# AlgoLab/rs-vgaligner

Measured on AMD Instinct MI355X. Metric: aligned reads/sec (10 kbp ONT vs HLA graph), higher is better.
Workload: dtype int32+f64

## Files before the change

rs-vgaligner_amd/csrc/vga_poa_t5.hpp:

```cpp
#pragma once

template <int B>
__device__ __forceinline__ void t5_min_byte(int &dst, int t, int c)
{
    if constexpr (B == 0) asm("v_min_u32_sdwa %0, %1, %2 dst_sel:BYTE_0 dst_unused:UNUSED_PRESERVE src0_sel:DWORD src1_sel:DWORD" : "+v"(dst) : "v"(t), "s"(c));
    if constexpr (B == 1) asm("v_min_u32_sdwa %0, %1, %2 dst_sel:BYTE_1 dst_unused:UNUSED_PRESERVE src0_sel:DWORD src1_sel:DWORD" : "+v"(dst) : "v"(t), "s"(c));
    if constexpr (B == 2) asm("v_min_u32_sdwa %0, %1, %2 dst_sel:BYTE_2 dst_unused:UNUSED_PRESERVE src0_sel:DWORD src1_sel:DWORD" : "+v"(dst) : "v"(t), "s"(c));
    if constexpr (B == 3) asm("v_min_u32_sdwa %0, %1, %2 dst_sel:BYTE_3 dst_unused:UNUSED_PRESERVE src0_sel:DWORD src1_sel:DWORD" : "+v"(dst) : "v"(t), "s"(c));
}
__device__ __forceinline__ uint64_t t5_uniform64(uint64_t v)
{
    return ((uint64_t)(uint32_t)__builtin_amdgcn_readfirstlane((int)(v >> 32)) << 32) | (uint32_t)__builtin_amdgcn_readfirstlane((int)(uint32_t)v);
}

__device__ __forceinline__ int t5_own(int v)
{
    asm volatile("" : "+v"(v));
    return __builtin_amdgcn_readfirstlane(v);
}
__device__ __forceinline__ uint32_t t5_own(uint32_t v) { return (uint32_t)t5_own((int)v); }
__device__ __forceinline__ uint64_t t5_own(uint64_t v) { return ((uint64_t)t5_own((uint32_t)(v >> 32)) << 32) | t5_own((uint32_t)v); }
template <typename T>
__device__ __forceinline__ T *t5_own(T *p) { return (T *)t5_own((uint64_t)p); }

#define POA_T5_ARGS_OFFSET 40
__device__ __forceinline__ const poa_t5_args *t5_kargs()
{
    uint32_t off = POA_T5_ARGS_OFFSET;
    asm volatile("" : "+s"(off));
    return (const poa_t5_args *)((const char *)__builtin_amdgcn_kernarg_segment_ptr() + off);
}
template <int NT, bool DEF>
__global__ __launch_bounds__(NT) __attribute__((amdgpu_waves_per_eu(5)))
void k_poa_dp_t5(const poa_prob *__restrict__ probs, const char *__restrict__ queries,
                                                       const uint4 *__restrict__ node_tab, const uint32_t *__restrict__ seq32,
                                                       const uint32_t *__restrict__ preds, const poa_t5_args A)
{
    poa_row *rows = A.rows;
    uint8_t *pool_arg = A.pool;
    const uint32_t lds_cols = t5_own(A.lds_cols), hg_cols = t5_own(A.hg_cols), win_mask = t5_own(A.win_mask);
    enum : uint32_t { ST_CHUNKED = 1u, ST_QPLAIN = 2u, ST_FAILED = 4u, ST_PREV_LDS = 8u, ST_PREV_FAR_USE = 16u };
    uint32_t st = (A.cp.n_slots != 0 ? ST_CHUNKED : 0u) | ST_PREV_LDS;
#define chunked ((st & ST_CHUNKED) != 0)
#define failed ((st & ST_FAILED) != 0)
#define q_plain ((st & ST_QPLAIN) != 0)
#define prev_lds ((st & ST_PREV_LDS) != 0)
#define prev_far_use ((st & ST_PREV_FAR_USE) != 0)
    struct { int match, mismatch, o1, e1, o2, e2, banded; } P = {t5_own(A.P.match), t5_own(A.P.mismatch), A.P.o1, A.P.e1, A.P.o2, A.P.e2, t5_own(A.P.banded)};
    constexpr int NW = NT / 64;
    constexpr int STEP = NT * 4;
    extern __shared__ __attribute__((aligned(16))) uint8_t smem[];
    int4 *sX = (int4 *)smem;
    int4 *sRed = sX + 2 * NW;
    int32_t *edgeW = (int32_t *)(sRed + NW);
    int32_t *sSink = edgeW + 4;
    uint64_t *sChunk = (uint64_t *)(sSink + 4);
    constexpr int HDR = (3 * NW + 1 + 1 + 2) * 16;
    int32_t *Hs = (int32_t *)(smem + HDR);
    uint16_t *Gs = (uint16_t *)(smem + HDR + 4ull * hg_cols);
    uint16_t *Qn = (uint16_t *)(smem + HDR + 6ull * hg_cols);
    const int edge_idx = (int)(edgeW - Hs);

    if (threadIdx.x == 0) A.outs[blockIdx.x].t_begin = __builtin_amdgcn_s_memrealtime();
    if (A.prio) __builtin_amdgcn_s_setprio(3);
    const poa_prob pb = probs[blockIdx.x];
    const int tid = threadIdx.x, lane = tid & 63, wv = __builtin_amdgcn_readfirstlane(tid >> 6);
    const int qlen = t5_own((int)pb.qlen);
    const char *query = queries + pb.q0;
    const uint4 *ntab = node_tab + t5_own(pb.node0);
    const uint32_t *plist = preds + t5_own(pb.pred0);
    const uint32_t *seqw = seq32 + t5_own(pb.seq0 >> 2);
    poa_row *R = rows + t5_own(pb.row0);
    const uint32_t n_nodes = t5_own(pb.n_nodes), ring_rows = t5_own(pb.ring_rows);

    uint8_t *pool = pool_arg;
    uint64_t state_lo = 0, state_hi = 0;
    if (chunked) {
        int got = -1;
        if (!(pb.flags & 1u)) {
            if (tid == 0) {
                got = poa_slot_acquire(A.cp.slot_flag, A.cp.n_slots, blockIdx.x);
                sSink[1] = got;
            }
            __syncthreads();
            got = __builtin_amdgcn_readfirstlane(sSink[1]);
        }
        if (got < 0) {
            if (tid == 0) {
                poa_out &O = A.outs[blockIdx.x];
                O.t_end = O.t_begin; O.cells = 0; O.vcells = 0; O.maxw = 0; O.nops = 0;
                O.score = POA_NEG; O.row = 0; O.status = POA_ST_POOL;
            }
            return;
        }
        __builtin_amdgcn_fence(__ATOMIC_ACQUIRE, "agent");
        pool = nullptr;
        state_lo = (uint64_t)A.cp.state_base + (uint64_t)(uint32_t)got * A.cp.state_size;
        state_hi = state_lo + A.cp.state_size;
    }

    const int o1 = DEF ? 4 : P.o1, e1 = DEF ? 2 : P.e1, o2 = DEF ? 24 : P.o2, e2 = DEF ? 1 : P.e2;
    const int C1 = 4 * (o1 + e1), C2 = 4 * (o2 + e2) + 1;
    const int D1 = 4 * o1, D2 = 4 * o2 + 1;
    const uint32_t g_bias = (uint32_t)(4 * e1 | (4 * e2) << 8) * 0x00010001u;
    const uint32_t e_probe = (uint32_t)((128 - D1) | (128 - D2) << 8) * 0x00010001u;
    const int bw = t5_own((int)pb.w);

    uint32_t own_head = POA_NIL, own_chunks = 0;
    auto alloc = [&](uint64_t &cur, uint32_t &rem, uint32_t bytes_asked, int slot) -> uint64_t {
        const uint32_t bytes = (bytes_asked + 15u) & ~15u;
        if (__builtin_expect(bytes > rem, 0)) {
            if (chunked) {
                if (slot == 0 && bytes <= POA_CHUNK) {
                    const poa_t5_args *ka = t5_kargs();
                    if (tid == 0) {
                        const uint32_t idx = poa_chunk_pop(ka->cp, blockIdx.x);
                        if (idx != POA_NIL) __hip_atomic_store(ka->cp.next + idx, own_head, __ATOMIC_RELAXED, __HIP_MEMORY_SCOPE_AGENT);
                        if (own_chunks == 0) sChunk[3] = idx;
                        sChunk[0] = idx;
                    }
                    __syncthreads();
                    const uint32_t idx = (uint32_t)__builtin_amdgcn_readfirstlane((int)(uint32_t)sChunk[0]);
                    __syncthreads();
                    if (idx == POA_NIL) st |= ST_FAILED;
// ... 70 lines not shown
        asm volatile("" : "+s"(st));
        POA_MARK("row_topo");
        const uint32_t r = nt.x + tn;
        const bool last = tn + 1 == nlen;
        const bool is_sink = last && (nt.z >> 31) != 0;
        const uint32_t ps = nt.w;
        uint32_t gb = 0;
        if (v > 0) {
            const uint32_t bi = r - 1;
            if ((bi & 3u) == 0 || (bi >> 2) != seq_word_idx) { seq_word_idx = bi >> 2; seq_word = seqw[seq_word_idx]; }
            gb = (seq_word >> (8u * (bi & 3u))) & 0xffu;
        }
        const bool simple = r > 0 && prev_lds && (tn > 0 || ((nt.y >> 24) == 1u && ps == r - 1));
        const bool writer = wv == (int)(r % (uint32_t)NW);
        POA_MARK("row_prevmax");
        int prev_lmax = 0, prev_rmax = 0;
        if (r > 0) {
            int4 rw = make_int4(INT32_MIN, INT32_MAX, INT32_MIN, 0);
            if (lane < NW) rw = sRed[lane];
            int b = rw.x, t;
            t = poa_dpp<0x111, 0xf>(INT32_MIN, b); b = t > b ? t : b;
            if (NW > 2) { t = poa_dpp<0x112, 0xf>(INT32_MIN, b); b = t > b ? t : b; }
            if (NW > 4) { t = poa_dpp<0x114, 0xf>(INT32_MIN, b); b = t > b ? t : b; }
            if (NW > 8) { t = poa_dpp<0x118, 0xf>(INT32_MIN, b); b = t > b ? t : b; }
            const int rbest = __builtin_amdgcn_readlane(b, NW - 1);
            const uint64_t tie = __builtin_amdgcn_ballot_w64(rw.x == rbest);
            if (__builtin_expect(__builtin_popcountll(tie) == 1, 1)) {
                const int w1 = __builtin_ctzll(tie);
                prev_lmax = __builtin_amdgcn_readlane(rw.y, w1);
                prev_rmax = __builtin_amdgcn_readlane(rw.z, w1);
            } else {
                int lm = rw.x == rbest ? rw.y : INT32_MAX, rm = rw.x == rbest ? rw.z : INT32_MIN;
                t = poa_dpp<0x111, 0xf>(INT32_MAX, lm); lm = t < lm ? t : lm;
                t = poa_dpp<0x111, 0xf>(INT32_MIN, rm); rm = t > rm ? t : rm;
                if (NW > 2) {
                    t = poa_dpp<0x112, 0xf>(INT32_MAX, lm); lm = t < lm ? t : lm;
                    t = poa_dpp<0x112, 0xf>(INT32_MIN, rm); rm = t > rm ? t : rm;
                }
                if (NW > 4) {
                    t = poa_dpp<0x114, 0xf>(INT32_MAX, lm); lm = t < lm ? t : lm;
                    t = poa_dpp<0x114, 0xf>(INT32_MIN, rm); rm = t > rm ? t : rm;
                }
                if (NW > 8) {
                    t = poa_dpp<0x118, 0xf>(INT32_MAX, lm); lm = t < lm ? t : lm;
                    t = poa_dpp<0x118, 0xf>(INT32_MIN, rm); rm = t > rm ? t : rm;
                }
                prev_lmax = __builtin_amdgcn_readlane(lm, NW - 1);
                prev_rmax = __builtin_amdgcn_readlane(rm, NW - 1);
            }
            if (prev_far_use && writer && lane == 0) { R[r - 1].lmax = prev_lmax; R[r - 1].rmax = prev_rmax; }
        }
        POA_MARK("row_setup");
        const int remain = (int)(nt.z & 0x3fffffffu) + (int)(nlen - 1 - tn);
        int beg, end, np, pbeg = prev_beg, pend = prev_end;
        bool first, single, sp_near;
        uint32_t sp = r - 1;
        uint64_t vpo = 0;
        if (__builtin_expect(simple, 1)) {
            first = tn == 0;
            np = 1; single = true; sp_near = true;
            const int mpl = prev_lmax + 1, mpr = prev_rmax + 1;
            if (!P.banded) { beg = 0; end = qlen; }
            else {
                const int diag = qlen - remain;
                const int lo = mpl < diag ? mpl : diag;
                const int hi = mpr > diag ? mpr : diag;
                beg = lo - bw; if (beg < 0) beg = 0;
                end = hi + bw; if (end > qlen) end = qlen;
            }
        } else {
            first = tn == 0 && v > 0;
            np = v == 0 ? 0 : (tn == 0 ? (int)(nt.y >> 24) : 1);
            bool far = r > 0 && !prev_lds;
            if (first) {
                if (np == 1) far |= ps != r - 1;
                else
                    for (int t = 0; t < np; t++) far |= plist[ps + t] != r - 1;
            }
            single = r > 0 && np == 1;
            sp = first ? ps : r - 1;
            sp_near = sp == r - 1 && prev_lds;
            if (far) __syncthreads();
            int mpl, mpr;
            if (r == 0) { mpl = 0; mpr = 0; }
            else if (!first) { mpl = prev_lmax + 1; mpr = prev_rmax + 1; }
            else {
                mpl = INT32_MAX; mpr = 0;
                for (int t = 0; t < np; t++) {
                    const uint32_t p = np == 1 ? ps : plist[ps + t];
                    int lm, rm;
                    if (p == r - 1) { lm = prev_lmax + 1; rm = prev_rmax + 1; }
                    else {
                        lm = __builtin_amdgcn_readfirstlane(R[p].lmax) + 1;
                        rm = __builtin_amdgcn_readfirstlane(R[p].rmax) + 1;
                    }
                    mpl = lm < mpl ? lm : mpl;
                    mpr = rm > mpr ? rm : mpr;
                }
            }
            if (!P.banded) { beg = 0; end = qlen; }
            else {
                const int diag = qlen - remain;
                const int lo = mpl < diag ? mpl : diag;
                const int hi = mpr > diag ? mpr : diag;
                beg = lo - bw; if (beg < 0) beg = 0;
                end = hi + bw; if (end > qlen) end = qlen;
            }
            if (single && !sp_near) {
                pbeg = __builtin_amdgcn_readfirstlane(R[sp].beg);
                pend = __builtin_amdgcn_readfirstlane(R[sp].end);
                vpo = t5_uniform64(R[sp].voff);
            }
        }
        const int bal = beg & ~3;
        const int W = (end - bal + 1 + 3) & ~3;
        const bool wide = (uint32_t)W + 8u > hg_cols;
        const bool keep = last || wide;
        const uint64_t doff = alloc(dcur, dend, (uint32_t)W * (np > 1 ? 4u : 1u), 0);
        uint64_t voff = 0;
        if (last && !failed) {
            if (r == 0 || (nt.z & 0x40000000u)) voff = chunked ? alloc(dcur, dend, 6u * (uint32_t)W, 0) : alloc(vcur, vendp, 6u * (uint32_t)W, 1);
            else {
                voff = ring_base + (uint64_t)ring_head * ((6u * (uint32_t)((qlen + 8) & ~3) + 15u) & ~15u);
                ring_head = ring_head + 1 == ring_rows ? 0 : ring_head + 1;
            }
        } else if (wide) voff = wide_scratch + (r & 1u) * 6ull * lds_cols;
        if (__builtin_expect(failed, 0)) break;
        if (writer && lane == 0) {
            uint32_t *rec = (uint32_t *)(R + r);
            *(uint4 *)rec = make_uint4((uint32_t)beg, (uint32_t)end, (uint32_t)doff, (uint32_t)(doff >> 32));
            *(uint2 *)(rec + 4) = make_uint2((uint32_t)voff, (uint32_t)(voff >> 32));
            *(HIP_vector_type<uint32_t, 3> *)(rec + 8) = HIP_vector_type<uint32_t, 3>(ps, first ? (uint32_t)np : 0u, keep ? 1u : 0u);
        }
        uint8_t *Vrow = pool + voff;
        uint8_t *drow = pool + doff;
        const uint32_t gd = gb - (uint32_t)'A';
        const bool acgt = gd < 20u && ((0x80045u >> gd) & 1u);
        const int sc_eq = acgt ? P.match : 0, sc_ne = acgt ? -P.mismatch : 0;
        const int gsh = (int)((gb >> 1) & 3u);
        const int ne4t = 4 * sc_ne + 1, mm4 = 4 * (sc_eq - sc_ne);
        const bool staged = !simple && r > 0 && !wide && q_plain;
        if (staged) {
            POA_MARK("row_stage");
            if (chunked) {
                bool no_row = false;
                for (int t = 0; t < np; t++) no_row |= t5_uniform64(R[np == 1 ? sp : plist[ps + t]].voff) == 0;
                if (__builtin_expect(no_row, 0)) st |= ST_FAILED;
            }
            for (int c0 = 0; c0 < W; c0 += STEP) {
                const int c = c0 + 4 * tid;
                const int j0 = bal + c;
                if (j0 <= end && np == 1) {
                    const int bp = __builtin_amdgcn_readfirstlane(R[sp].beg), ep = __builtin_amdgcn_readfirstlane(R[sp].end);
                    const uint64_t vq_off = t5_uniform64(R[sp].voff);
                    const uint8_t *Vq = pool + vq_off;
                    const bool vq_ok = !chunked || vq_off != 0;
                    const int balq = bp & ~3;
                    const int Wq = (ep - balq + 1 + 3) & ~3;
                    const int idx = j0 - balq;
                    int4 hv = make_int4(T4_NEG, T4_NEG, T4_NEG, T4_NEG);
                    uint2 gg = make_uint2(0u, 0u);
                    if (idx >= 0 && idx < Wq && vq_ok) {
                        hv = *(const int4 *)((const int32_t *)Vq + idx);
                        gg = *(const uint2 *)(Vq + 4ll * Wq + 2ll * idx);
                    }
                    const unsigned pspan = (unsigned)(ep - bp);
                    const bool in0 = (unsigned)(j0 - bp) <= pspan, in1 = (unsigned)(j0 + 1 - bp) <= pspan, in2 = (unsigned)(j0 + 2 - bp) <= pspan,
                               in3 = (unsigned)(j0 + 3 - bp) <= pspan;
                    hv.x = in0 ? hv.x : T4_NEG; hv.y = in1 ? hv.y : T4_NEG; hv.z = in2 ? hv.z : T4_NEG; hv.w = in3 ? hv.w : T4_NEG;
                    gg.x = (in0 ? gg.x & 0xffffu : 0u) | (in1 ? gg.x & 0xffff0000u : 0u);
                    gg.y = (in2 ? gg.y & 0xffffu : 0u) | (in3 ? gg.y & 0xffff0000u : 0u);
                    *(int4 *)(Hs + (j0 & win_mask)) = hv;
                    *(uint2 *)(Gs + (j0 & win_mask)) = gg;
                    if (c == 0 && bal > 0) {
                        const int wl = (idx >= 1 && idx - 1 < Wq && vq_ok) ? ((const int32_t *)Vq)[idx - 1] : 0;
                        Hs[(bal - 1) & win_mask] = (unsigned)(j0 - 1 - bp) <= pspan ? wl : T4_NEG;
                    }
                } else if (j0 <= end) {
                    int hm[4], x1[4], x2[4], ah[4], a1[4], a2[4];
                    int hl = T4_NEG, ahl = 0;
#pragma unroll
                    for (int k = 0; k < 4; k++) { hm[k] = T4_NEG; x1[k] = T4_NEG; x2[k] = T4_NEG; ah[k] = 0; a1[k] = 0; a2[k] = 0; }
                    for (int t = 0; t < np; t++) {
                        const uint32_t p = np == 1 ? sp : plist[ps + t];
                        const int bp = __builtin_amdgcn_readfirstlane(R[p].beg), ep = __builtin_amdgcn_readfirstlane(R[p].end);
                        const uint64_t vq_off = t5_uniform64(R[p].voff);
                        const uint8_t *Vq = pool + vq_off;
                        const int balq = bp & ~3;
                        const int Wq = (!chunked || vq_off != 0) ? (ep - balq + 1 + 3) & ~3 : 0;
                        const int idx = j0 - balq;
                        int4 hv = make_int4(0, 0, 0, 0);
                        uint2 gg = make_uint2(0u, 0u);
                        if (idx >= 0 && idx < Wq) {
                            hv = *(const int4 *)((const int32_t *)Vq + idx);
                            gg = *(const uint2 *)(Vq + 4ll * Wq + 2ll * idx);
                        }
                        int wl = (idx >= 1 && idx - 1 < Wq) ? ((const int32_t *)Vq)[idx - 1] : 0;
                        const unsigned pspan = (unsigned)(ep - bp);
                        const int hj[4] = {hv.x, hv.y, hv.z, hv.w};
                        const uint32_t g16[4] = {gg.x & 0xffffu, gg.x >> 16, gg.y & 0xffffu, gg.y >> 16};
#pragma unroll
                        for (int k = 0; k < 4; k++) {
                            if ((unsigned)(j0 + k - bp) <= pspan) {
                                const int h = hj[k], c1 = h - (int)(g16[k] & 255u), c2 = h - (int)(g16[k] >> 8);
                                if (h > hm[k]) { hm[k] = h; ah[k] = t; }
                                if (c1 > x1[k]) { x1[k] = c1; a1[k] = t; }
                                if (c2 > x2[k]) { x2[k] = c2; a2[k] = t; }
                            }
                        }
                        if (j0 >= 1 && (unsigned)(j0 - 1 - bp) <= pspan && wl > hl) { hl = wl; ahl = t; }
                    }
                    const int4 hq = make_int4(hm[0], hm[1], hm[2], hm[3]);
                    uint32_t gv[4];
#pragma unroll
                    for (int k = 0; k < 4; k++) gv[k] = (uint32_t)(hm[k] - x1[k]) | ((uint32_t)(hm[k] - x2[k]) << 8);
                    *(int4 *)(Hs + (j0 & win_mask)) = hq;
                    *(uint2 *)(Gs + (j0 & win_mask)) = make_uint2(gv[0] | (gv[1] << 16), gv[2] | (gv[3] << 16));
                    if (c == 0 && bal > 0) Hs[(bal - 1) & win_mask] = hl;
                    if (np > 1) {
                        *(uint32_t *)(drow + (uint64_t)W + c) = (uint32_t)ahl | ((uint32_t)ah[0] << 8) | ((uint32_t)ah[1] << 16) | ((uint32_t)ah[2] << 24);
                        *(uint32_t *)(drow + 2ull * W + c) = (uint32_t)a1[0] | ((uint32_t)a1[1] << 8) | ((uint32_t)a1[2] << 16) | ((uint32_t)a1[3] << 24);
                        *(uint32_t *)(drow + 3ull * W + c) = (uint32_t)a2[0] | ((uint32_t)a2[1] << 8) | ((uint32_t)a2[2] << 16) | ((uint32_t)a2[3] << 24);
                    }
                }
            }
            POA_LDS_BARRIER();
            pbeg = bal > 0 ? bal - 1 : 0;
            pend = bal + W - 1;
        }
        const uint8_t *Vp = pool + vpo;
        const int balp = pbeg & ~3;

        POA_MARK("row_steps");
        enum : uint32_t { F_SINGLE = 1u, F_NEAR = 2u, F_PLAIN = 4u, F_WIDE = 8u, F_KEEP = 16u, F_SINK = 32u, F_MULTI = 64u, F_SRC = 128u };
        const uint32_t rowf = (single ? F_SINGLE : 0u) | (sp_near ? F_NEAR : 0u) | (q_plain ? F_PLAIN : 0u) | (wide ? F_WIDE : 0u) |
                              (keep ? F_KEEP : 0u) | (is_sink ? F_SINK : 0u) | (np > 1 ? F_MULTI : 0u) | (r == 0 ? F_SRC : 0u);
        int best = INT32_MIN, lpos = beg, rpos = beg;
        const bool hot = (simple || staged) && !wide && q_plain;
        const int rlim = end < pend ? end : pend;
        auto run_steps = [&](auto hot_c) __attribute__((always_inline)) {
        constexpr bool HOT = decltype(hot_c)::value;
        int carry1 = POA_IDENT, carry2 = POA_IDENT, left1 = POA_IDENT, left2 = POA_IDENT;
        int next_left = 0;
        int buf = 0;
        for (int c0 = 0; c0 < W; c0 += STEP, buf ^= 1) {
            uint32_t f = HOT ? (rowf & (F_KEEP | F_SINK)) : rowf;
            asm volatile("" : "+s"(f));
            if (HOT) f |= F_SINGLE | F_NEAR | F_PLAIN;
            const int c = c0 + 4 * tid;
            const int j0 = bal + c;
            const bool lane_act = j0 <= end;
            const int jw0 = bal + c0 + 256 * wv, jw1 = jw0 + 255;
            const bool wave_act = jw0 <= end;
            int d_lp = jw0 - beg, d_rp = rlim - jw1, d_lq = (jw0 > beg ? jw0 : beg) - pbeg - 1;
            asm volatile("" : "+s"(d_lp), "+s"(d_rp), "+s"(d_lq));
            const uint32_t e_lp = (uint32_t)d_lp >> 31;
            const uint32_t e_rp = (uint32_t)d_rp >> 31;
            const uint32_t e_lq = (uint32_t)d_lq >> 31;
            const bool lp = e_lp != 0, rp = e_rp != 0, lq = e_lq != 0;
            int htt[4], ht4[4], e1t[4], e2t[4], pmeta[4];
            int agg1 = POA_IDENT, agg2 = POA_IDENT, alast1 = POA_IDENT, alast2 = POA_IDENT;
#pragma unroll
            for (int k = 0; k < 4; k++) { htt[k] = T4_NEG + 2; ht4[k] = T4_NEG; e1t[k] = T4_NEG + 1; e2t[k] = T4_NEG; pmeta[k] = 0; }
            uint32_t qn = 0u;
            if (wave_act) qn = (uint32_t)Qn[j0 >> 2];
            const bool fastw = HOT ? wave_act
                                   : (f & (F_SINGLE | F_PLAIN)) == (F_SINGLE | F_PLAIN) && wave_act && (!lq || (f & F_NEAR)) && (!rp || ((f & F_NEAR) && end <= pend + 1));
            const int base1 = 4 * e1 * j0, base2 = 4 * e2 * j0;
        if constexpr (HOT) POA_MARK("hot_p1_fast"); else POA_MARK("p1_fast");
            if (__builtin_expect(fastw, 1)) {
                int4 hv;
                uint2 gg;
                int hprev;
                if constexpr (HOT) {
                    hv = *(const int4 *)(Hs + (j0 & win_mask));
                    gg = *(const uint2 *)(Gs + (j0 & win_mask));
                    int left0;
                    if (wv == 0 && c0 > 0) left0 = next_left;
                    else left0 = Hs[(jw0 > 0 ? jw0 - 1 : 0) & (int)win_mask];
                    if (wv == 0 && c0 + STEP < W) next_left = Hs[(jw0 + STEP - 1) & (int)win_mask];
                    hprev = t4_shr1_mov(hv.w, left0);
                } else if (__builtin_expect((f & F_NEAR) != 0, 1)) {
                    hv = *(const int4 *)(Hs + (j0 & win_mask));
                    gg = *(const uint2 *)(Gs + (j0 & win_mask));
                    if (tid == NT - 1) edgeW[buf] = hv.w;
                    {
                        const bool edge = tid == 0 && c0 > 0;
                        int w = Hs[edge ? edge_idx + (buf ^ 1) : ((j0 > 0 ? j0 - 1 : 0) & win_mask)];
                        asm volatile("" : "+v"(w));
                        hprev = w;
                    }
                } else {
                    const int Wp = (pend - balp + 1 + 3) & ~3;
                    const int idx = j0 - balp;
                    hv = *(const int4 *)((const int32_t *)Vp + idx);
                    gg = *(const uint2 *)(Vp + 4ll * Wp + 2ll * idx);
                    hprev = ((const int32_t *)Vp)[idx > 0 ? idx - 1 : 0];
                    asm volatile("" : "+v"(hv.x), "+v"(hv.y), "+v"(hv.z), "+v"(hv.w), "+v"(gg.x), "+v"(gg.y), "+v"(hprev));
                }
                auto phase1 = [&](auto edge_c) {
                    constexpr bool EDGE = decltype(edge_c)::value;
                    int hj[4] = {hv.x, hv.y, hv.z, hv.w};
                    int ga = (int)gg.x, gbb = (int)gg.y;
                    if constexpr (EDGE) {
                        if (rp) {
#pragma unroll
                            for (int k = 0; k < 4; k++) hj[k] = j0 + k > pend ? T4_NEG : hj[k];
                            ga = j0 > pend ? 0 : (j0 + 1 > pend ? (ga & 0xffff) : ga);
                            gbb = j0 + 2 > pend ? 0 : (j0 + 3 > pend ? (gbb & 0xffff) : gbb);
                        }
                        if (lq) {
#pragma unroll
                            for (int k = 0; k < 4; k++) hj[k] = j0 + k < pbeg ? T4_NEG : hj[k];
                            ga = j0 + 1 < pbeg ? 0 : (j0 < pbeg ? (int)((uint32_t)ga & 0xffff0000u) : ga);
                            gbb = j0 + 3 < pbeg ? 0 : (j0 + 2 < pbeg ? (int)((uint32_t)gbb & 0xffff0000u) : gbb);
                        }
                    }
                    const uint32_t eqb = qn >> gsh;
                    int hp = hprev;
                    if constexpr (EDGE && HOT) {
                        if (rp) hp = j0 - 1 > pend ? T4_NEG : hp;
                    }
#pragma unroll
                    for (int k = 0; k < 4; k++) {
                        const int g = k < 2 ? ga : gbb;
                        const int ev1 = (k & 1) ? t4_sub_byte<2>(hj[k], g) : t4_sub_byte<0>(hj[k], g);
                        const int ev2 = (k & 1) ? t4_sub_byte<3>(hj[k], g) : t4_sub_byte<1>(hj[k], g);
                        int m = (int)__umul24(__builtin_amdgcn_ubfe(eqb, 4u * k, 1u), (uint32_t)mm4) + (hp + ne4t);
                        if constexpr (EDGE) {
                            if (lq) m = j0 + k - 1 < pbeg ? T4_NEG + 2 : m;
                        }
                        const int h = t4_max3(m, ev1, ev2);
                        htt[k] = h;
                        ht4[k] = h & ~3;
                        e1t[k] = ev1;
                        e2t[k] = ev2;
                        hp = hj[k];
                    }
                    if constexpr (EDGE) {
                        if (lp) {
#pragma unroll
                            for (int k = 0; k < 4; k++) ht4[k] = j0 + k < beg ? POA_IDENT : ht4[k];
                        }
                    }
                    const int r11 = ht4[1] + 4 * e1, r12 = ht4[2] + 8 * e1, r13 = ht4[3] + 12 * e1;
                    const int r21 = ht4[1] + 4 * e2, r22 = ht4[2] + 8 * e2, r23 = ht4[3] + 12 * e2;
                    const int a1 = t4_max3(ht4[0], r11, r12), a2 = t4_max3(ht4[0], r21, r22);
                    agg1 = (a1 > r13 ? a1 : r13) + base1;
                    agg2 = (a2 > r23 ? a2 : r23) + base2;
                    alast1 = r13 + base1;
                    alast2 = r23 + base2;
                };
                if (__builtin_expect((e_lp | e_rp | e_lq) != 0, 0)) phase1(std::true_type{});
                else phase1(std::false_type{});
        if constexpr (HOT) POA_MARK("hot_p1_lean"); else POA_MARK("p1_lean");
            } else if (wave_act && (f & F_SINGLE)) {
                int pbeg_ = pbeg, pend_ = pend, beg_ = beg, end_ = end, balp_ = balp, gsh_ = gsh;
                asm volatile("" : "+s"(pbeg_), "+s"(pend_), "+s"(beg_), "+s"(end_), "+s"(balp_), "+s"(gsh_));
                const int pbeg = pbeg_, pend = pend_, beg = beg_, end = end_, balp = balp_, gsh = gsh_;
                const unsigned span = (unsigned)(end - beg), pspan = (unsigned)(pend - pbeg);
                int hj[4], wm0;
                uint32_t g16[4];
                if (f & F_NEAR) {
                    const int4 hv = *(const int4 *)(Hs + (j0 & win_mask));
                    const uint2 gg = *(const uint2 *)(Gs + (j0 & win_mask));
                    hj[0] = hv.x; hj[1] = hv.y; hj[2] = hv.z; hj[3] = hv.w;
                    g16[0] = gg.x & 0xffffu; g16[1] = gg.x >> 16; g16[2] = gg.y & 0xffffu; g16[3] = gg.y >> 16;
                    if (tid == NT - 1) edgeW[buf] = hj[3];
                    const bool edge = tid == 0 && c0 > 0;
                    int w = Hs[edge ? edge_idx + (buf ^ 1) : ((j0 > 0 ? j0 - 1 : 0) & win_mask)];
                    asm volatile("" : "+v"(w));
                    wm0 = w;
                } else {
                    const int idx = j0 - balp;
                    const int Wp = (pend - balp + 1 + 3) & ~3;
                    int4 hv = make_int4(0, 0, 0, 0);
                    uint2 gg = make_uint2(0u, 0u);
                    if (idx >= 0 && idx < Wp) {
                        hv = *(const int4 *)((const int32_t *)Vp + idx);
                        gg = *(const uint2 *)(Vp + 4ll * Wp + 2ll * idx);
                    }
                    wm0 = (idx >= 1 && idx - 1 < Wp) ? ((const int32_t *)Vp)[idx - 1] : 0;
                    asm volatile("" : "+v"(hv.x), "+v"(hv.y), "+v"(hv.z), "+v"(hv.w), "+v"(gg.x), "+v"(gg.y), "+v"(wm0));
                    hj[0] = hv.x; hj[1] = hv.y; hj[2] = hv.z; hj[3] = hv.w;
                    g16[0] = gg.x & 0xffffu; g16[1] = gg.x >> 16; g16[2] = gg.y & 0xffffu; g16[3] = gg.y >> 16;
                }
                bool inprev = j0 >= 1 && (unsigned)(j0 - 1 - pbeg) <= pspan;
#pragma unroll
                for (int k = 0; k < 4; k++) {
                    const int j = j0 + k;
                    const bool inj = (unsigned)(j - pbeg) <= pspan;
                    const bool actk = (unsigned)(j - beg) <= span;
                    const int qc = (int)((qn >> (4 * k)) & 15u);
                    const int s = ((qc >> gsh) & 1) ? sc_eq : (qc == 0 ? 0 : sc_ne);
                    const int wm = k == 0 ? wm0 : hj[k - 1];
                    const int m = inprev ? wm + 4 * s + 1 : T4_NEG + 2;
                    const int ev1 = inj ? hj[k] - (int)(g16[k] & 255u) : T4_NEG + 1;
                    const int ev2 = inj ? hj[k] - (int)(g16[k] >> 8) : T4_NEG;
                    const int h = t4_max3(m, ev1, ev2);
                    htt[k] = h;
                    ht4[k] = h & ~3;
                    e1t[k] = ev1;
                    e2t[k] = ev2;
                    const int a1 = actk ? ht4[k] + 4 * e1 * j : POA_IDENT, a2 = actk ? ht4[k] + 4 * e2 * j : POA_IDENT;
                    agg1 = a1 > agg1 ? a1 : agg1;
                    agg2 = a2 > agg2 ? a2 : agg2;
                    if (k == 3) { alast1 = a1; alast2 = a2; }
                    inprev = inj;
                }
        if constexpr (HOT) POA_MARK("hot_p1_general"); else POA_MARK("p1_general");
            } else if (wave_act) {
                int beg_ = beg, end_ = end, gsh_ = gsh;
                asm volatile("" : "+s"(beg_), "+s"(end_), "+s"(gsh_));
                const int beg = beg_, end = end_, gsh = gsh_;
                const unsigned span = (unsigned)(end - beg);
                if (f & F_SRC) {
#pragma unroll
                    for (int k = 0; k < 4; k++) { ht4[k] = (j0 + k == 0) ? 0 : T4_NEG; htt[k] = ht4[k] + 2; }
                } else if (lane_act) {
                    int m[4], ev1[4], ev2[4];
#pragma unroll
                    for (int k = 0; k < 4; k++) { m[k] = T4_NEG + 2; ev1[k] = T4_NEG + 1; ev2[k] = T4_NEG; }
                    for (int t = 0; t < np; t++) {
                        const uint32_t p = plist[ps + t];
                        int hj[4], wm0 = 0;
                        uint32_t g16[4];
                        int bp, ep;
                        if (p == r - 1 && prev_lds) {
                            bp = prev_beg; ep = prev_end;
                            const int4 hv = *(const int4 *)(Hs + (j0 & win_mask));
                            const uint2 gg = *(const uint2 *)(Gs + (j0 & win_mask));
                            hj[0] = hv.x; hj[1] = hv.y; hj[2] = hv.z; hj[3] = hv.w;
                            g16[0] = gg.x & 0xffffu; g16[1] = gg.x >> 16; g16[2] = gg.y & 0xffffu; g16[3] = gg.y >> 16;
                            if (tid == NT - 1) edgeW[buf] = hj[3];
                            const bool edge = tid == 0 && c0 > 0;
                            int w = Hs[edge ? edge_idx + (buf ^ 1) : ((j0 > 0 ? j0 - 1 : 0) & win_mask)];
                            asm volatile("" : "+v"(w));
                            wm0 = w;
                        } else {
                            bp = __builtin_amdgcn_readfirstlane(R[p].beg);
                            ep = __builtin_amdgcn_readfirstlane(R[p].end);
                            const uint64_t vo = R[p].voff;
                            const uint64_t vos = ((uint64_t)(uint32_t)__builtin_amdgcn_readfirstlane((int)(vo >> 32)) << 32) |
                                                 (uint32_t)__builtin_amdgcn_readfirstlane((int)(uint32_t)vo);
                            const uint8_t *Vq = pool + vos;
                            const int balq = bp & ~3;
                            const int Wq = (ep - balq + 1 + 3) & ~3;
                            const int idx = j0 - balq;
                            int4 hv = make_int4(0, 0, 0, 0);
                            uint2 gg = make_uint2(0u, 0u);
                            if (idx >= 0 && idx < Wq) {
                                hv = *(const int4 *)((const int32_t *)Vq + idx);
                                gg = *(const uint2 *)(Vq + 4ll * Wq + 2ll * idx);
                            }
                            wm0 = (idx >= 1 && idx - 1 < Wq) ? ((const int32_t *)Vq)[idx - 1] : 0;
                            asm volatile("" : "+v"(hv.x), "+v"(hv.y), "+v"(hv.z), "+v"(hv.w), "+v"(gg.x), "+v"(gg.y), "+v"(wm0));
                            hj[0] = hv.x; hj[1] = hv.y; hj[2] = hv.z; hj[3] = hv.w;
                            g16[0] = gg.x & 0xffffu; g16[1] = gg.x >> 16; g16[2] = gg.y & 0xffffu; g16[3] = gg.y >> 16;
                        }
                        const unsigned pspan = (unsigned)(ep - bp);
#pragma unroll
                        for (int k = 0; k < 4; k++) {
                            const int j = j0 + k;
                            const bool actk = (unsigned)(j - beg) <= span;
                            const int qc = (int)((qn >> (4 * k)) & 15u);
                            const int s = ((qc >> gsh) & 1) ? sc_eq : (qc == 0 ? 0 : sc_ne);
                            const int wm = k == 0 ? wm0 : hj[k - 1];
                            if (actk && j >= 1 && (unsigned)(j - 1 - bp) <= pspan) {
                                const int cnd = wm + 4 * s + 1;
                                if (cnd > m[k]) { m[k] = cnd; pmeta[k] = (pmeta[k] & ~255) | t; }
                            }
                            if (actk && (unsigned)(j - bp) <= pspan) {
                                const int c1 = hj[k] - (int)(g16[k] & 255u);
                                if (c1 > ev1[k]) { ev1[k] = c1; pmeta[k] = (pmeta[k] & ~0xff00) | (t << 8); }
                                const int c2 = hj[k] - (int)(g16[k] >> 8);
                                if (c2 > ev2[k]) { ev2[k] = c2; pmeta[k] = (pmeta[k] & ~0xff0000) | (t << 16); }
                            }
                        }
                    }
#pragma unroll
                    for (int k = 0; k < 4; k++) {
                        const int h = t4_max3(m[k], ev1[k], ev2[k]);
                        htt[k] = h;
                        ht4[k] = h & ~3;
                        e1t[k] = ev1[k];
                        e2t[k] = ev2[k];
                    }
                }
#pragma unroll
                for (int k = 0; k < 4; k++) {
                    const int j = j0 + k;
                    const bool actk = (unsigned)(j - beg) <= span;
                    const int a1 = actk ? ht4[k] + 4 * e1 * j : POA_IDENT, a2 = actk ? ht4[k] + 4 * e2 * j : POA_IDENT;
                    agg1 = a1 > agg1 ? a1 : agg1;
                    agg2 = a2 > agg2 ? a2 : agg2;
                    if (k == 3) { alast1 = a1; alast2 = a2; }
                }
            }
        if constexpr (HOT) POA_MARK("hot_scan"); else POA_MARK("scan");
            int i1 = POA_IDENT, i2 = POA_IDENT;
            if (wave_act) {
                i1 = poa_wave_scan_max(agg1);
                i2 = poa_wave_scan_max(agg2);
            }
            if (lane == 63) sX[buf * NW + wv] = make_int4(i1, i2, alast1, alast2);
            POA_LDS_BARRIER();
        if constexpr (HOT) POA_MARK("hot_exchange"); else POA_MARK("exchange");
            int pre1 = carry1, pre2 = carry2, pl1 = left1, pl2 = left2;
            {
                const bool more = c0 + STEP < W;
                if ((wave_act && wv > 0) || more) {
                    int4 x = make_int4(POA_IDENT, POA_IDENT, POA_IDENT, POA_IDENT);
                    if (lane < NW) x = sX[buf * NW + lane];
                    int s1 = x.x, s2 = x.y, t;
                    t = poa_dpp<0x111, 0xf>(INT32_MIN, s1); s1 = t > s1 ? t : s1;
                    t = poa_dpp<0x111, 0xf>(INT32_MIN, s2); s2 = t > s2 ? t : s2;
                    if (NW > 2) {
                        t = poa_dpp<0x112, 0xf>(INT32_MIN, s1); s1 = t > s1 ? t : s1;
                        t = poa_dpp<0x112, 0xf>(INT32_MIN, s2); s2 = t > s2 ? t : s2;
                    }
                    if (NW > 4) {
                        t = poa_dpp<0x114, 0xf>(INT32_MIN, s1); s1 = t > s1 ? t : s1;
                        t = poa_dpp<0x114, 0xf>(INT32_MIN, s2); s2 = t > s2 ? t : s2;
                    }
                    if (NW > 8) {
                        t = poa_dpp<0x118, 0xf>(INT32_MIN, s1); s1 = t > s1 ? t : s1;
                        t = poa_dpp<0x118, 0xf>(INT32_MIN, s2); s2 = t > s2 ? t : s2;
                    }
                    if (wv > 0) {
                        const int a = __builtin_amdgcn_readlane(s1, wv - 1), b = __builtin_amdgcn_readlane(s2, wv - 1);
                        pre1 = a > pre1 ? a : pre1;
                        pre2 = b > pre2 ? b : pre2;
                        pl1 = __builtin_amdgcn_readlane(x.z, wv - 1);
                        pl2 = __builtin_amdgcn_readlane(x.w, wv - 1);
                    }
                    if (more) {
                        const int a = __builtin_amdgcn_readlane(s1, NW - 1), b = __builtin_amdgcn_readlane(s2, NW - 1);
                        carry1 = a > carry1 ? a : carry1;
                        carry2 = b > carry2 ? b : carry2;
                        left1 = __builtin_amdgcn_readlane(x.z, NW - 1);
                        left2 = __builtin_amdgcn_readlane(x.w, NW - 1);
                    }
                }
            }
            if (wave_act) {
                const int run1_ = t4_shr1_max(i1, pre1), run2_ = t4_shr1_max(i2, pre2);
                const int la1_ = t4_shr1_mov(alast1, pl1), la2_ = t4_shr1_mov(alast2, pl2);
        if constexpr (HOT) POA_MARK("hot_p2_fast"); else POA_MARK("p2_fast");
                if (__builtin_expect(fastw, 1)) {
                    auto phase2 = [&](auto edge_c) {
                        constexpr bool EDGE = decltype(edge_c)::value;
                        int R1 = run1_ - base1, R2 = run2_ - base2, L1 = la1_ - base1, L2 = la2_ - base2;
                        int h4[4];
                        int dirq = 0, ga = 0, gbb = 0;
#pragma unroll
                        for (int k = 0; k < 4; k++) {
                            const int f1 = R1 - (4 * (o1 + e1 * k) - 1), f2 = R2 - 4 * (o2 + e2 * k);
                            const int hh = t4_max3(ht4[k] | 3, f1, f2);
                            const int h = (hh & ~3) | 1;
                            h4[k] = h;
                            int acc = (hh << 2) | (htt[k] & 3);
                            const int u1 = h - e1t[k], u2 = h - e2t[k];
                            if (k == 0) { t5_min_byte<0>(ga, u1, D1); t5_min_byte<1>(ga, u2, D2); }
                            if (k == 1) { t5_min_byte<2>(ga, u1, D1); t5_min_byte<3>(ga, u2, D2); }
                            if (k == 2) { t5_min_byte<0>(gbb, u1, D1); t5_min_byte<1>(gbb, u2, D2); }
                            if (k == 3) { t5_min_byte<2>(gbb, u1, D1); t5_min_byte<3>(gbb, u2, D2); }
                            t4_flag_ne(acc, R1, L1);
                            if (k == 0) t4_flag_ne_dep<0>(dirq, acc, R2, L2);
                            if (k == 1) t4_flag_ne_dep<1>(dirq, acc, R2, L2);
                            if (k == 2) t4_flag_ne_dep<2>(dirq, acc, R2, L2);
                            if (k == 3) t4_flag_ne_dep<3>(dirq, acc, R2, L2);
                            L1 = ht4[k] + 4 * e1 * k; L2 = ht4[k] + 4 * e2 * k;
                            R1 = L1 > R1 ? L1 : R1;
                            R2 = L2 > R2 ? L2 : R2;
                        }
                        {
                            const uint32_t ya = (uint32_t)ga + e_probe, yb = ((uint32_t)gbb + e_probe) >> 1;
                            const uint32_t e8 = (ya & 0x80808080u) | (yb & ~0x80808080u);
                            dirq = (int)((e8 & 0xC0C0C0C0u) | ((uint32_t)dirq & ~0xC0C0C0C0u));
                            ga = (int)((uint32_t)ga + g_bias);
                            gbb = (int)((uint32_t)gbb + g_bias);
                        }
                        {
                            int hb[4] = {h4[0], h4[1], h4[2], h4[3]};
                            if constexpr (EDGE) {
#pragma unroll
                                for (int k = 0; k < 4; k++) hb[k] = j0 + k > end ? INT32_MIN : hb[k];
                            }
                            const int m3 = t4_max3(hb[0], hb[1], hb[2]);
                            const int m4 = m3 > hb[3] ? m3 : hb[3];
                            if (m4 >= best) {
                                const int kf = hb[0] == m4 ? 0 : (hb[1] == m4 ? 1 : (hb[2] == m4 ? 2 : 3));
                                const int kl = hb[3] == m4 ? 3 : (hb[2] == m4 ? 2 : (hb[1] == m4 ? 1 : 0));
                                if (m4 > best) { best = m4; lpos = j0 + kf; }
                                rpos = j0 + kl;
                            }
                        }
                        if (__builtin_expect((f & F_SINK) != 0, 0)) {
                            const int kq = qlen - j0;
#pragma unroll
                            for (int k = 0; k < 4; k++)
                                if (kq == k) sSink[0] = h4[k];
                        }
                        if (!EDGE || j0 <= end) {
                            const int4 hq = make_int4(h4[0], h4[1], h4[2], h4[3]);
                            const uint2 gq = make_uint2((uint32_t)ga, (uint32_t)gbb);
                            if (!(f & F_WIDE)) {
                                *(int4 *)(Hs + (j0 & win_mask)) = hq;
                                *(uint2 *)(Gs + (j0 & win_mask)) = gq;
                            }
                            *(uint32_t *)(drow + c) = (uint32_t)dirq;
                            if (f & F_KEEP) {
                                *(int4 *)((int32_t *)Vrow + c) = hq;
                                *(uint2 *)(Vrow + 4ll * W + 2ll * c) = gq;
                            }
                        }
                    };
                    if (__builtin_expect((e_lp | e_rp) != 0, 0)) phase2(std::true_type{});
                    else phase2(std::false_type{});
        if constexpr (HOT) POA_MARK("hot_p2_slow"); else POA_MARK("p2_slow");
                } else if (lane_act) {
                    int beg_ = beg, end_ = end;
                    asm volatile("" : "+s"(beg_), "+s"(end_));
                    const int beg = beg_;
                    const unsigned span = (unsigned)(end_ - beg_);
                    int run1 = run1_, run2 = run2_, la1 = la1_, la2 = la2_;
                    int h4[4];
                    uint32_t g16[4], codev[4];
#pragma unroll
                    for (int k = 0; k < 4; k++) {
                        const int j = j0 + k;
                        const bool actk = (unsigned)(j - beg) <= span;
                        const int f1 = run1 - 4 * (o1 + e1 * j) + 1, f2 = run2 - 4 * (o2 + e2 * j);
                        const int hh = t4_max3(ht4[k] | 3, f1, f2);
                        const int h = (hh & ~3) | 1;
                        h4[k] = h;
                        const uint32_t t1 = (uint32_t)((h + 4 * e1) - e1t[k]), t2 = (uint32_t)((h + 4 * e2) - e2t[k]);
                        const uint32_t G1 = t1 < (uint32_t)C1 ? t1 : (uint32_t)C1, G2 = t2 < (uint32_t)C2 ? t2 : (uint32_t)C2;
                        g16[k] = G1 | (G2 << 8);
                        codev[k] = (((uint32_t)(hh & 3) << 4) | ((uint32_t)(htt[k] & 3) << 2) | (run1 != la1 ? 2u : 0u) | (run2 != la2 ? 1u : 0u)) << (8 * k);
                        codev[k] |= ((t1 >= (uint32_t)C1 ? 1u : 0u) | (t2 >= (uint32_t)C2 ? 256u : 0u)) << (16 * (k & 1) + (k < 2 ? 7 : 6));
                        const int hb = actk ? h : INT32_MIN;
                        if (hb > best) { best = hb; lpos = j; rpos = j; }
                        else if (actk && hb == best) rpos = j;
                        const int a1 = actk ? ht4[k] + 4 * e1 * j : POA_IDENT, a2 = actk ? ht4[k] + 4 * e2 * j : POA_IDENT;
                        run1 = a1 > run1 ? a1 : run1;
                        run2 = a2 > run2 ? a2 : run2;
                        la1 = actk ? a1 : la1; la2 = actk ? a2 : la2;
                    }
                    if (__builtin_expect((f & F_SINK) != 0, 0)) {
                        const int kq = qlen - j0;
#pragma unroll
                        for (int k = 0; k < 4; k++)
                            if (kq == k) sSink[0] = h4[k];
                    }
                    const int Wl = (end_ - bal + 1 + 3) & ~3;
                    {
                        const int4 hq = make_int4(h4[0], h4[1], h4[2], h4[3]);
                        const uint2 gq = make_uint2(g16[0] | (g16[1] << 16), g16[2] | (g16[3] << 16));
                        if (!(f & F_WIDE)) {
                            *(int4 *)(Hs + (j0 & win_mask)) = hq;
                            *(uint2 *)(Gs + (j0 & win_mask)) = gq;
                        }
                        *(uint32_t *)(drow + c) = codev[0] | codev[1] | codev[2] | codev[3];
                        if (f & F_KEEP) {
                            *(int4 *)((int32_t *)Vrow + c) = hq;
                            *(uint2 *)(Vrow + 4ll * Wl + 2ll * c) = gq;
                        }
                        if (__builtin_expect((f & F_MULTI) != 0, 0)) {
                            *(uint32_t *)(drow + (uint64_t)Wl + c) = (uint32_t)(pmeta[0] & 255) | ((uint32_t)(pmeta[1] & 255) << 8) | ((uint32_t)(pmeta[2] & 255) << 16) | ((uint32_t)(pmeta[3] & 255) << 24);
                            *(uint32_t *)(drow + 2ull * Wl + c) = (uint32_t)((pmeta[0] >> 8) & 255) | ((uint32_t)((pmeta[1] >> 8) & 255) << 8) | ((uint32_t)((pmeta[2] >> 8) & 255) << 16) | ((uint32_t)((pmeta[3] >> 8) & 255) << 24);
                            *(uint32_t *)(drow + 3ull * Wl + c) = (uint32_t)((pmeta[0] >> 16) & 255) | ((uint32_t)((pmeta[1] >> 16) & 255) << 8) | ((uint32_t)((pmeta[2] >> 16) & 255) << 16) | ((uint32_t)((pmeta[3] >> 16) & 255) << 24);
                        }
                    }
                }
            }
        if constexpr (HOT) POA_MARK("hot_step_end"); else POA_MARK("step_end");
        }
        };
        if (__builtin_expect(hot, 1)) run_steps(std::true_type{});
        else run_steps(std::false_type{});
        POA_MARK("row_reduce");
        {
            const int wb = __builtin_amdgcn_readlane(poa_wave_scan_max(best), 63);
            const bool mine = best == wb;
            const uint64_t tie = __builtin_amdgcn_ballot_w64(mine);
            int *red = (int *)(sRed + wv);
            if (__builtin_expect(__builtin_popcountll(tie) == 1, 1)) {
                if (mine) { red[0] = best; red[1] = lpos; red[2] = rpos; }
            } else {
                int lm = mine ? lpos : INT32_MAX, rm = mine ? rpos : INT32_MIN;
                lm = poa_wave_scan_min(lm);
                rm = poa_wave_scan_max(rm);
                if (lane == 63) { red[0] = wb; red[1] = lm; red[2] = rm; }
            }
        }
        POA_LDS_BARRIER();
        POA_MARK("row_end");
        if (__builtin_expect(is_sink, 0) && tid == 0) {
            const int val = (qlen >= beg && qlen <= end) ? sSink[0] >> 2 : POA_NEG;
            if (sSink[3] == 0 || val > sSink[2]) { sSink[2] = val; sSink[3] = (int)r + 1; }
        }
        prev_beg = beg; prev_end = end;
        st = (st & ~(ST_PREV_LDS | ST_PREV_FAR_USE)) | (wide ? 0u : ST_PREV_LDS) | (last ? ST_PREV_FAR_USE : 0u);
    }
    }
    POA_MARK("epilogue");
    __syncthreads();
    if (tid >= 64) return;
    const poa_t5_args E = *t5_kargs();
    const poa_prob pe = E.probs[blockIdx.x];
    poa_out &O = E.outs[blockIdx.x];
    int status = POA_ST_OK;
    uint32_t start_row = 0;
    int sink_best = POA_NEG;
    if (failed) status = POA_ST_POOL;
    else {
        sink_best = __builtin_amdgcn_readfirstlane(sSink[2]);
        const int sr = __builtin_amdgcn_readfirstlane(sSink[3]);
        start_row = sr ? (uint32_t)(sr - 1) : 0u;
        status = (sr != 0 && sink_best > POA_NEG / 2) ? POA_ST_OK : POA_ST_NOALN;
        const poa_row *Rr = E.rows + pe.row0;
        uint64_t cells = 0, vcells = 0;
        int maxw = 0;
        for (uint32_t r = (uint32_t)lane; r <= pe.N; r += 64) {
            const int b = Rr[r].beg, e = Rr[r].end, kp = Rr[r].base;
            const int W = (e - (b & ~3) + 1 + 3) & ~3;
            maxw = W > maxw ? W : maxw;
            if (r > 0) cells += (uint64_t)(e - b + 1);
            if (kp) vcells += (uint64_t)(e - b + 1);
        }
        for (int sh = 32; sh > 0; sh >>= 1) {
            cells += __shfl_down(cells, sh);
            vcells += __shfl_down(vcells, sh);
            const int m2 = __shfl_down(maxw, sh);
            maxw = m2 > maxw ? m2 : maxw;
        }
        if (tid == 0) { O.cells = cells; O.vcells = vcells; O.maxw = (uint32_t)maxw; }
    }
    if (tid == 0) {
        if (failed) { O.cells = 0; O.vcells = 0; O.maxw = 0; }
        O.score = failed ? POA_NEG : sink_best;
        O.row = start_row;
        O.status = status;
    }
    if (E.tb_ops) {
        uint8_t *pool_e = E.cp.n_slots ? nullptr : E.pool;
        poa_traceback_wave<2>(*(tb_lds *)(smem + HDR), tid, pe, E.rows, E.preds, pool_e, O, E.tb_ops, E.tb_orow, 0, status, start_row);
    }
    if (tid == 0) {
        O.t_end = __builtin_amdgcn_s_memrealtime();
        if (E.cp.n_slots) {
            const uint32_t state_slot = (uint32_t)sSink[1];
            if (own_head != POA_NIL) poa_chunk_push(E.cp, blockIdx.x, own_head, (uint32_t)sChunk[3]);
            const uint64_t state_lo = (uint64_t)E.cp.state_base + (uint64_t)state_slot * E.cp.state_size;
            (void)atomicAdd(E.pool_next, (unsigned long long)own_chunks * POA_CHUNK + (vcur - state_lo));
            __builtin_amdgcn_fence(__ATOMIC_RELEASE, "agent");
            (void)atomicExch(&E.cp.slot_flag[state_slot], 0u);
        }
    }
}
#undef chunked
#undef failed
#undef q_plain
#undef prev_lds
#undef prev_far_use
```

Before: 10580.

## Add fast staging paths for single far predecessor and two-predecessor merge rows

Row staging gains a fast interior path. Rows with one far predecessor copy its H/G values straight into the LDS window. Rows with exactly two predecessors, one of them the previous LDS-resident row, merge the two sources in a dedicated staging pass that also writes the per-predecessor argmax bytes. Predecessor row metadata (beg/end/voff/lmax/rmax) is loaded once with vector loads and hoisted out of the per-step loop. Writing the multi-predecessor metadata moves from the hot step epilogue into the general multi-pred branch, which cuts register pressure and branches in the hot loop, at the cost of more code and extra LDS barriers.

```diff
diff --git a/rs-vgaligner_amd/csrc/vga_poa_t5.hpp b/rs-vgaligner_amd/csrc/vga_poa_t5.hpp
--- a/rs-vgaligner_amd/csrc/vga_poa_t5.hpp
+++ b/rs-vgaligner_amd/csrc/vga_poa_t5.hpp
@@ -39,7 +39,8 @@
     poa_row *rows = A.rows;
     uint8_t *pool_arg = A.pool;
     const uint32_t lds_cols = t5_own(A.lds_cols), hg_cols = t5_own(A.hg_cols), win_mask = t5_own(A.win_mask);
-    enum : uint32_t { ST_CHUNKED = 1u, ST_QPLAIN = 2u, ST_FAILED = 4u, ST_PREV_LDS = 8u, ST_PREV_FAR_USE = 16u };
+    enum : uint32_t { ST_CHUNKED = 1u, ST_QPLAIN = 2u, ST_FAILED = 4u, ST_PREV_LDS = 8u, ST_PREV_FAR_USE = 16u,
+                      ST_MERGE2 = 32u, ST_NEAR1 = 64u };
     uint32_t st = (A.cp.n_slots != 0 ? ST_CHUNKED : 0u) | ST_PREV_LDS;
 #define chunked ((st & ST_CHUNKED) != 0)
 #define failed ((st & ST_FAILED) != 0)
@@ -276,9 +277,32 @@
             sp_near = sp == r - 1 && prev_lds;
             if (far) __syncthreads();
             int mpl, mpr;
+            uint32_t pf = ps;
+            bool one_far = first && np == 1 && ps != r - 1;
+            if (first && np == 2 && prev_lds) {
+                const uint32_t p0 = plist[ps], p1 = plist[ps + 1];
+                if ((p0 == r - 1) != (p1 == r - 1)) {
+                    st |= p1 == r - 1 ? ST_MERGE2 | ST_NEAR1 : ST_MERGE2;
+                    pf = p0 == r - 1 ? p1 : p0;
+                    one_far = true;
+                }
+            }
             if (r == 0) { mpl = 0; mpr = 0; }
             else if (!first) { mpl = prev_lmax + 1; mpr = prev_rmax + 1; }
-            else {
+            else if (one_far) {
+                const uint32_t *rec = (const uint32_t *)(R + pf);
+                const uint2 ra = *(const uint2 *)rec;
+                const uint4 rb = *(const uint4 *)(rec + 4);
+                pbeg = __builtin_amdgcn_readfirstlane((int)ra.x);
+                pend = __builtin_amdgcn_readfirstlane((int)ra.y);
+                vpo = ((uint64_t)(uint32_t)__builtin_amdgcn_readfirstlane((int)rb.y) << 32) | (uint32_t)__builtin_amdgcn_readfirstlane((int)rb.x);
+                mpl = __builtin_amdgcn_readfirstlane((int)rb.z) + 1;
+                mpr = __builtin_amdgcn_readfirstlane((int)rb.w) + 1;
+                if (np == 2) {
+                    mpl = prev_lmax + 1 < mpl ? prev_lmax + 1 : mpl;
+                    mpr = prev_rmax + 1 > mpr ? prev_rmax + 1 : mpr;
+                }
+            } else {
                 mpl = INT32_MAX; mpr = 0;
                 for (int t = 0; t < np; t++) {
                     const uint32_t p = np == 1 ? ps : plist[ps + t];
@@ -300,7 +324,7 @@
                 beg = lo - bw; if (beg < 0) beg = 0;
                 end = hi + bw; if (end > qlen) end = qlen;
             }
-            if (single && !sp_near) {
+            if (single && !sp_near && !one_far) {
                 pbeg = __builtin_amdgcn_readfirstlane(R[sp].beg);
                 pend = __builtin_amdgcn_readfirstlane(R[sp].end);
                 vpo = t5_uniform64(R[sp].voff);
@@ -336,21 +360,102 @@
         const bool staged = !simple && r > 0 && !wide && q_plain;
         if (staged) {
             POA_MARK("row_stage");
+            const bool one_rec = np == 1 || (st & ST_MERGE2) != 0;
             if (chunked) {
                 bool no_row = false;
-                for (int t = 0; t < np; t++) no_row |= t5_uniform64(R[np == 1 ? sp : plist[ps + t]].voff) == 0;
+                if (one_rec) no_row = vpo == 0;
+                else
+                    for (int t = 0; t < np; t++) no_row |= t5_uniform64(R[plist[ps + t]].voff) == 0;
                 if (__builtin_expect(no_row, 0)) st |= ST_FAILED;
+            }
+            int fb = pbeg, fe = pend;
+            uint32_t vq_lo = (uint32_t)vpo, vq_hi = (uint32_t)(vpo >> 32);
+            asm volatile("" : "+s"(fb), "+s"(fe), "+s"(vq_lo), "+s"(vq_hi));
+            const uint64_t vq_off = (uint64_t)vq_hi << 32 | vq_lo;
+            const bool vq_ok = !chunked || vq_off != 0;
+            const uint8_t *Vq = pool + vq_off;
+            const int balq = fb & ~3;
+            const int Wq = (fe - balq + 1 + 3) & ~3;
+            int ilo = INT32_MAX, ihi = INT32_MIN;
+            if (one_rec && vq_ok) {
+                ilo = fb; ihi = fe;
+                if (np == 2) { ilo = prev_beg > ilo ? prev_beg : ilo; ihi = prev_end < ihi ? prev_end : ihi; }
+            }
+            int near_left = 0;
+            if (st & ST_MERGE2) {
+                int ln = lane;
+                asm volatile("" : "+v"(ln));
+                const int cs = bal + ln * STEP + 256 * wv;
+                if (cs > 0 && cs <= end) near_left = Hs[(cs - 1) & (int)win_mask];
+                POA_LDS_BARRIER();
+            }
+            int si = 0;
+            for (int c0 = 0; c0 < W; c0 += STEP, si++) {
+                const int c = c0 + 4 * tid;
+                const int j0 = bal + c;
+                const int jw0 = bal + c0 + 256 * wv;
+                const bool interior = jw0 - 1 >= ilo && jw0 + 255 <= ihi;
+                if (interior && np == 1) {
+                    const int idx = j0 - balq;
+                    const int4 hv = *(const int4 *)((const int32_t *)Vq + idx);
+                    const uint2 gg = *(const uint2 *)(Vq + 4ll * Wq + 2ll * idx);
+                    if (j0 <= end) {
+                        *(int4 *)(Hs + (j0 & win_mask)) = hv;
+                        *(uint2 *)(Gs + (j0 & win_mask)) = gg;
+                        if (c == 0) Hs[(bal - 1) & win_mask] = ((const int32_t *)Vq)[idx - 1];
+                    }
+                } else if (interior) {
+                    POA_MARK("stage_merge");
+                    const int idx = j0 - balq;
+                    const int4 hf = *(const int4 *)((const int32_t *)Vq + idx);
+                    const uint2 gf = *(const uint2 *)(Vq + 4ll * Wq + 2ll * idx);
+                    const int wlf = ((const int32_t *)Vq)[idx - 1];
+                    const int4 hn = *(const int4 *)(Hs + (j0 & win_mask));
+                    const uint2 gn = *(const uint2 *)(Gs + (j0 & win_mask));
+                    const int wln = t4_shr1_mov(hn.w, __builtin_amdgcn_readlane(near_left, si));
+                    auto merge = [&](const int4 hA, const uint2 gA, const int wA, const int4 hB, const uint2 gB, const int wB) __attribute__((always_inline)) {
+                        const int ha[4] = {hA.x, hA.y, hA.z, hA.w}, hb[4] = {hB.x, hB.y, hB.z, hB.w};
+                        int hm[4];
+                        uint32_t gv[4], ah[4], a1[4], a2[4];
+                        int neg = T4_NEG;
+                        asm volatile("" : "+s"(neg));
+#pragma unroll
+                        for (int k = 0; k < 4; k++) {
+                            const int wa = (int)(k < 2 ? gA.x : gA.y), wb = (int)(k < 2 ? gB.x : gB.y);
+                            const int c1a = (k & 1) ? t4_sub_byte<2>(ha[k], wa) : t4_sub_byte<0>(ha[k], wa);
+                            const int c2a = (k & 1) ? t4_sub_byte<3>(ha[k], wa) : t4_sub_byte<1>(ha[k], wa);
+                            const int c1b = (k & 1) ? t4_sub_byte<2>(hb[k], wb) : t4_sub_byte<0>(hb[k], wb);
+                            const int c2b = (k & 1) ? t4_sub_byte<3>(hb[k], wb) : t4_sub_byte<1>(hb[k], wb);
+                            const int mh = ha[k] > neg ? ha[k] : neg, m1 = c1a > neg ? c1a : neg, m2 = c2a > neg ? c2a : neg;
+                            ah[k] = (uint32_t)(mh - hb[k]) >> 31; a1[k] = (uint32_t)(m1 - c1b) >> 31; a2[k] = (uint32_t)(m2 - c2b) >> 31;
+                            hm[k] = hb[k] > mh ? hb[k] : mh;
+                            const int x1 = c1b > m1 ? c1b : m1, x2 = c2b > m2 ? c2b : m2;
+                            gv[k] = (uint32_t)(hm[k] - x1) | ((uint32_t)(hm[k] - x2) << 8);
+                        }
+                        const int ml = wA > neg ? wA : neg;
+                        const uint32_t ahl = (uint32_t)(ml - wB) >> 31;
+                        const int hl = wB > ml ? wB : ml;
+                        if (j0 <= end) {
+                            *(int4 *)(Hs + (j0 & win_mask)) = make_int4(hm[0], hm[1], hm[2], hm[3]);
+                            *(uint2 *)(Gs + (j0 & win_mask)) = make_uint2(gv[0] | (gv[1] << 16), gv[2] | (gv[3] << 16));
+                            if (c == 0) Hs[(bal - 1) & win_mask] = hl;
+                            *(uint32_t *)(drow + (uint64_t)W + c) = ahl | (ah[0] << 8) | (ah[1] << 16) | (ah[2] << 24);
+                            *(uint32_t *)(drow + 2ull * W + c) = a1[0] | (a1[1] << 8) | (a1[2] << 16) | (a1[3] << 24);
+                            *(uint32_t *)(drow + 3ull * W + c) = a2[0] | (a2[1] << 8) | (a2[2] << 16) | (a2[3] << 24);
+                        }
+                    };
+                    if (st & ST_NEAR1) merge(hf, gf, wlf, hn, gn, wln);
+                    else merge(hn, gn, wln, hf, gf, wlf);
+                }
             }
             for (int c0 = 0; c0 < W; c0 += STEP) {
                 const int c = c0 + 4 * tid;
                 const int j0 = bal + c;
+                const int jw0 = bal + c0 + 256 * wv;
+                if (jw0 - 1 >= ilo && jw0 + 255 <= ihi) continue;
+                POA_MARK("stage_general");
                 if (j0 <= end && np == 1) {
-                    const int bp = __builtin_amdgcn_readfirstlane(R[sp].beg), ep = __builtin_amdgcn_readfirstlane(R[sp].end);
-                    const uint64_t vq_off = t5_uniform64(R[sp].voff);
-                    const uint8_t *Vq = pool + vq_off;
-                    const bool vq_ok = !chunked || vq_off != 0;
-                    const int balq = bp & ~3;
-                    const int Wq = (ep - balq + 1 + 3) & ~3;
+                    const int bp = fb, ep = fe;
                     const int idx = j0 - balq;
                     int4 hv = make_int4(T4_NEG, T4_NEG, T4_NEG, T4_NEG);
                     uint2 gg = make_uint2(0u, 0u);
@@ -452,10 +557,10 @@
             const uint32_t e_rp = (uint32_t)d_rp >> 31;
             const uint32_t e_lq = (uint32_t)d_lq >> 31;
             const bool lp = e_lp != 0, rp = e_rp != 0, lq = e_lq != 0;
-            int htt[4], ht4[4], e1t[4], e2t[4], pmeta[4];
+            int htt[4], ht4[4], e1t[4], e2t[4];
             int agg1 = POA_IDENT, agg2 = POA_IDENT, alast1 = POA_IDENT, alast2 = POA_IDENT;
 #pragma unroll
-            for (int k = 0; k < 4; k++) { htt[k] = T4_NEG + 2; ht4[k] = T4_NEG; e1t[k] = T4_NEG + 1; e2t[k] = T4_NEG; pmeta[k] = 0; }
+            for (int k = 0; k < 4; k++) { htt[k] = T4_NEG + 2; ht4[k] = T4_NEG; e1t[k] = T4_NEG + 1; e2t[k] = T4_NEG; }
             uint32_t qn = 0u;
             if (wave_act) qn = (uint32_t)Qn[j0 >> 2];
             const bool fastw = HOT ? wave_act
@@ -612,9 +717,9 @@
 #pragma unroll
                     for (int k = 0; k < 4; k++) { ht4[k] = (j0 + k == 0) ? 0 : T4_NEG; htt[k] = ht4[k] + 2; }
                 } else if (lane_act) {
-                    int m[4], ev1[4], ev2[4];
-#pragma unroll
-                    for (int k = 0; k < 4; k++) { m[k] = T4_NEG + 2; ev1[k] = T4_NEG + 1; ev2[k] = T4_NEG; }
+                    int m[4], ev1[4], ev2[4], pmeta[4];
+#pragma unroll
+                    for (int k = 0; k < 4; k++) { m[k] = T4_NEG + 2; ev1[k] = T4_NEG + 1; ev2[k] = T4_NEG; pmeta[k] = 0; }
                     for (int t = 0; t < np; t++) {
                         const uint32_t p = plist[ps + t];
                         int hj[4], wm0 = 0;
@@ -680,6 +785,12 @@
                         e1t[k] = ev1[k];
                         e2t[k] = ev2[k];
                     }
+                    if (f & F_MULTI) {
+                        const int Wl = (end - bal + 1 + 3) & ~3;
+                        *(uint32_t *)(drow + (uint64_t)Wl + c) = (uint32_t)(pmeta[0] & 255) | ((uint32_t)(pmeta[1] & 255) << 8) | ((uint32_t)(pmeta[2] & 255) << 16) | ((uint32_t)(pmeta[3] & 255) << 24);
+                        *(uint32_t *)(drow + 2ull * Wl + c) = (uint32_t)((pmeta[0] >> 8) & 255) | ((uint32_t)((pmeta[1] >> 8) & 255) << 8) | ((uint32_t)((pmeta[2] >> 8) & 255) << 16) | ((uint32_t)((pmeta[3] >> 8) & 255) << 24);
+                        *(uint32_t *)(drow + 3ull * Wl + c) = (uint32_t)((pmeta[0] >> 16) & 255) | ((uint32_t)((pmeta[1] >> 16) & 255) << 8) | ((uint32_t)((pmeta[2] >> 16) & 255) << 16) | ((uint32_t)((pmeta[3] >> 16) & 255) << 24);
+                    }
                 }
 #pragma unroll
                 for (int k = 0; k < 4; k++) {
@@ -806,7 +917,7 @@
                             *(uint32_t *)(drow + c) = (uint32_t)dirq;
                             if (f & F_KEEP) {
                                 *(int4 *)((int32_t *)Vrow + c) = hq;
-                                *(uint2 *)(Vrow + 4ll * W + 2ll * c) = gq;
+                                *(uint2 *)(Vrow + (uint32_t)(4 * W + 2 * c)) = gq;
                             }
                         }
                     };
@@ -861,11 +972,6 @@
                             *(int4 *)((int32_t *)Vrow + c) = hq;
                             *(uint2 *)(Vrow + 4ll * Wl + 2ll * c) = gq;
                         }
-                        if (__builtin_expect((f & F_MULTI) != 0, 0)) {
-                            *(uint32_t *)(drow + (uint64_t)Wl + c) = (uint32_t)(pmeta[0] & 255) | ((uint32_t)(pmeta[1] & 255) << 8) | ((uint32_t)(pmeta[2] & 255) << 16) | ((uint32_t)(pmeta[3] & 255) << 24);
-                            *(uint32_t *)(drow + 2ull * Wl + c) = (uint32_t)((pmeta[0] >> 8) & 255) | ((uint32_t)((pmeta[1] >> 8) & 255) << 8) | ((uint32_t)((pmeta[2] >> 8) & 255) << 16) | ((uint32_t)((pmeta[3] >> 8) & 255) << 24);
-                            *(uint32_t *)(drow + 3ull * Wl + c) = (uint32_t)((pmeta[0] >> 16) & 255) | ((uint32_t)((pmeta[1] >> 16) & 255) << 8) | ((uint32_t)((pmeta[2] >> 16) & 255) << 16) | ((uint32_t)((pmeta[3] >> 16) & 255) << 24);
-                        }
                     }
                 }
             }
@@ -896,7 +1002,7 @@
             if (sSink[3] == 0 || val > sSink[2]) { sSink[2] = val; sSink[3] = (int)r + 1; }
         }
         prev_beg = beg; prev_end = end;
-        st = (st & ~(ST_PREV_LDS | ST_PREV_FAR_USE)) | (wide ? 0u : ST_PREV_LDS) | (last ? ST_PREV_FAR_USE : 0u);
+        st = (st & ~(ST_PREV_LDS | ST_PREV_FAR_USE | ST_MERGE2 | ST_NEAR1)) | (wide ? 0u : ST_PREV_LDS) | (last ? ST_PREV_FAR_USE : 0u);
     }
     }
     POA_MARK("epilogue");
```

New measurement: 10450. -1.3%, worse.
